# KTH-RPL/HiMo

Hardware: AMD Instinct MI355X
Metric: lidar_frames_per_sec_120k (higher is better)
Workload: dtype f16x2 (two-term split fp16, x = h + l with exact subnormals, on the matrix cores; float32 accumulate; ~22-bit products); 1 GPU; per-frame pipeline: pillarise 3 sweeps (512x512 grid) -> SeFlow++-style encoder/decoder + GRU head (random-init, self-specified: reference network source absent) -> per-point flow -> ego-motion removal + dt0 + flow2compDis -> comp_dis; points_per_frame=120000, sweeps_per_frame=3, parallelism=frames sharded x1, refined_output=False, batches_in_flight=3, matrix_arithmetic=f16x2, samples_per_backbone_launch=16, collectives=none (single process)

## Files before the change

### himo_amd/csrc/conv_common.h

```cpp
#pragma once
#include "himo_common.h"
#include "bf16x3.h"
#include <math.h>

namespace himo {

typedef float floatx16 __attribute__((ext_vector_type(16)));

enum Epilogue {
    kEpiBias = 0,
    kEpiBiasBnGelu = 1,
    kEpiBiasGelu = 2,
    kEpiGruZR = 3,
    kEpiGruQ = 4,
    kEpiBiasRelu = 5,
    kEpiReluMask = 6
};

struct ConvArgs {
    const float* x; int64_t x_batch_stride; int x_pitch;
    const float* w;
    const float* bias; const float* scale; const float* shift;
    float* y; int64_t y_batch_stride; int y_pitch;
    int N, H, W, Cin, Cout;
    int n_inner; int64_t x_outer_stride, y_outer_stride;
    int Ho, Wo;
    const float* aux_in; int aux_in_pitch;
    float* aux_out; int aux_out_pitch;
    int act_flags;
    unsigned* range_seen;
    const unsigned long long* mask;
    int64_t mask_batch_stride, mask_outer_stride;
};
enum ActFlags { kActSplitIn = 1, kActSplitOut = 2, kActVecStore = 4, kActAccumulate = 8, kActStuffedIn = 16, kActRowMask = 32 };

__device__ inline int64_t image_offset(int img, int n_inner, int64_t batch_stride, int64_t outer_stride) {
    return (int64_t)(img % n_inner) * batch_stride + (int64_t)(img / n_inner) * outer_stride;
}

__device__ inline int xcd_block_id(int bid, int n_blocks) {
    const int per = n_blocks >> 3, rem = n_blocks & 7;
    const int xcd = bid & 7, idx = bid >> 3;
    return xcd * per + (xcd < rem ? xcd : rem) + idx;
}

__device__ inline float gelu_exact(float v) {
    const float hv = 0.5f * v;
    const float t = __builtin_amdgcn_rcpf(fmaf(0.3275911f * 0.70710678118654752440f, fabsf(v), 1.0f));
    float p = fmaf(1.061405429f, t, -1.453152027f);
    p = fmaf(p, t, 1.421413741f);
    p = fmaf(p, t, -0.284496736f);
    p = fmaf(p, t, 0.254829592f);
    const float ex = __builtin_amdgcn_exp2f((v * v) * (-0.5f * 1.44269504088896340736f));
    const float e = fmaf(-(p * t), ex, 1.0f);
    return fmaf(fabsf(hv), e, hv);
// ... 55 lines not shown

__device__ inline unsigned split_word(float v, bool odd);
template <int EPI, bool PAIRED>
__device__ inline void split_store(const ConvArgs& a, float* __restrict__ yout, int64_t pix, int co, float v, float sc, float sh) {
    if (EPI == kEpiBiasBnGelu) v = gelu_exact(v * sc + sh);
    else if (EPI == kEpiBiasGelu) v = gelu_exact(v);
    else if (EPI == kEpiBiasRelu) v = fmaxf(v, 0.f);
    if (PAIRED) {
        const bool odd = co & 1;
        unsigned* rec = reinterpret_cast<unsigned*>(yout + pix * a.y_pitch + (co & ~15));
        rec[(odd ? 8 : 0) + ((co & 15) >> 1)] = split_word(v, odd);
        return;
    }
    unsigned h, l;
    split2_rounded(v, h, l);
    {
        unsigned short* rec = reinterpret_cast<unsigned short*>(yout + pix * a.y_pitch + (co & ~15));
        rec[co & 15] = (unsigned short)h;
        rec[16 + (co & 15)] = (unsigned short)l;
    }
}

constexpr float kSplitRangeGuard = 0.015625f;
__device__ inline void note_range(const ConvArgs& a, float v) {
    if (a.range_seen && __ballot(fabsf(v) >= kSplitRangeGuard) != 0ull && (threadIdx.x & 63) == 0 &&
        __hip_atomic_load(a.range_seen, __ATOMIC_RELAXED, __HIP_MEMORY_SCOPE_AGENT) == 0u)
        __hip_atomic_store(a.range_seen, 1u, __ATOMIC_RELAXED, __HIP_MEMORY_SCOPE_AGENT);
}

inline bool vec_store_ok(const ConvArgs& a) {
    return (reinterpret_cast<uintptr_t>(a.y) & 15u) == 0 && !(a.y_pitch & 3) && !(a.y_batch_stride & 3) && !(a.y_outer_stride & 3) && !(a.Cout & 3) &&
           (int64_t)a.Ho * a.Wo * a.y_pitch < ((int64_t)1 << 29);
}

template <bool OSPLIT, bool MASK = false, bool ACC = false>
__device__ inline void store_block_vec(const ConvArgs& a, float* __restrict__ yout, unsigned char* stg, const unsigned (&word)[16],
                                       int lane, int64_t pix0, int n_valid_px, int ch0) {
    const int li = lane & 31, lh = lane >> 5;
    const int widx = OSPLIT ? (li >> 4) * 16 + ((li & 1) ? 8 : 0) + ((li & 15) >> 1) : li;
#pragma unroll
    for (int r = 0; r < 16; ++r) {
        const int px = (r & 3) + 8 * (r >> 2) + 4 * lh;
        const int slot = px ^ ((px >> 2) & 1);
        *reinterpret_cast<unsigned*>(stg + slot * 128 + widx * 4) = word[r];
    }
    __builtin_amdgcn_wave_barrier();
#pragma unroll
    for (int t = 0; t < 4; ++t) {
        const int q = t * 64 + lane;
        const int slot = q >> 3, piece = q & 7;
        const int px = slot ^ ((slot >> 2) & 1);
// ... 34 lines not shown
```

### himo_amd/csrc/conv_plan.h

```cpp
#pragma once
#include "conv_common.h"

namespace himo {

enum ConvFamily {
    kConvF32,
    kConvStaged,
    kConvFromL2,
    kConvPresplit3,
    kConvPresplit1
};

struct ConvPlan {
    ConvFamily family;
    ConvArgs args;
    int ks, stride, epi, fmt;
    int bn, mi, ph, nt;
    const void* w_packed;
    dim3 grid;
    const char* prof_name;
};

void launch_conv_f32(const ConvPlan& p, hipStream_t s);
void launch_conv_staged(const ConvPlan& p, hipStream_t s);
void launch_conv_from_l2(const ConvPlan& p, hipStream_t s);
void launch_conv_presplit3(const ConvPlan& p, hipStream_t s);
void launch_conv_presplit1(const ConvPlan& p, hipStream_t s);

inline int64_t blocks_for(const ConvArgs& a, int th, int tw, int bn) {
    const int64_t tiles = th ? (int64_t)((a.Ho + th - 1) / th) * ((a.Wo + tw - 1) / tw) : ((int64_t)a.Ho * a.Wo + tw - 1) / tw;
    return (int64_t)a.N * tiles * ((a.Cout + bn - 1) / bn);
}

inline bool below_2gb(int64_t pixels, int pitch) { return pixels * pitch * 4 < ((int64_t)1 << 31); }

inline const char* conv_prof_name(int ks, int stride, int fmt) {
    static const char* const names[3][4] = {
        {"conv1x1_mfma_kernel", "conv1x1_bf16x3_kernel", "conv1x1_f16x2_kernel", "conv1x1_bf16x2_kernel"},
        {"conv3x3_mfma_kernel", "conv3x3_bf16x3_kernel", "conv3x3_f16x2_kernel", "conv3x3_bf16x2_kernel"},
        {"conv3x3s2_mfma_kernel", "conv3x3s2_bf16x3_kernel", "conv3x3s2_f16x2_kernel", "conv3x3s2_bf16x2_kernel"}};
    return names[ks == 1 ? 0 : stride == 2 ? 2 : 1][fmt < 0 ? 0 : fmt == 1 ? 2 : fmt == 2 ? 3 : 1];
}

// ... 38 lines not shown
    if (vec && (!(a.act_flags & kActSplitOut) || !(a.Cout & 15))) a.act_flags |= kActVecStore;
    return true;
}

inline int plan_presplit(ConvPlan& p, int rows_hint) {
    ConvArgs& a = p.args;
    if (!below_2gb((int64_t)a.H * a.W, a.x_pitch)) return HIMO_ERR_UNSUPPORTED;
    if (a.act_flags & kActRowMask) {
        p.family = kConvPresplit3;
        p.prof_name = "conv3x3_masked_f16x2_kernel";
        plan_rows_tile(p, 4, 2, 2);
        return HIMO_OK;
    }
    const bool wide = a.Cout > 64, vec = vec_store_ok(a), pinned = rows_hint == 4 || rows_hint == 2 || rows_hint == 1;
    const int ph = wide ? 1 : 2;
    p.family = p.ks == 1 ? kConvPresplit1 : kConvPresplit3;
    p.prof_name = conv_prof_name(p.ks, p.stride, 1);
    if (vec) a.act_flags |= kActVecStore;
    if (p.ks == 1) {
        int mi = wide ? 4 : 2;
        while (mi > 1 && blocks_for(a, 0, mi * ph * 32, (4 / ph) * 32) < 2048) mi >>= 1;
        if (pinned) mi = rows_hint;
        plan_rows_tile(p, ph, !wide && mi == 4 ? 2 : mi, 1);
    } else if (p.stride == 2) {
        plan_rows_tile(p, ph, wide ? 2 : 1, 1);
    } else if (!wide && rows_hint == 8 && vec) {
        plan_rows_tile(p, 4, 2, 2);
    } else if (wide && rows_hint == 12 && vec) {
        plan_rows_tile(p, a.Cout % 256 == 0 ? 1 : 2, 4, 2);
    } else {
        int mi = blocks_for(a, 4 * ph, 32, (4 / ph) * 32) >= 1024 ? 4 : 2;
        if (pinned) mi = rows_hint;
        plan_rows_tile(p, ph, !wide && mi == 4 ? 2 : mi, 1);
    }
    return HIMO_OK;
}

inline int plan_conv(const himo_conv_desc& d, ConvPlan& p) {
    if (!d.x || !d.w || !d.y) return HIMO_ERR_INVALID_ARGUMENT;
    if (d.n < 1 || d.h < 1 || d.w_in < 1 || d.cin < 1 || d.cout < 1) return HIMO_ERR_INVALID_ARGUMENT;
    if (!(d.ksize == 1 || d.ksize == 3) || !(d.stride == 1 || d.stride == 2)) return HIMO_ERR_UNSUPPORTED;
    if (d.ksize == 1 && d.stride != 1) return HIMO_ERR_UNSUPPORTED;
    if (d.epilogue < 0 || d.epilogue > kEpiReluMask) return HIMO_ERR_INVALID_ARGUMENT;
    if (d.epilogue == kEpiBiasBnGelu && (!d.scale || !d.shift)) return HIMO_ERR_INVALID_ARGUMENT;
    const bool gru = d.epilogue == kEpiGruZR || d.epilogue == kEpiGruQ;
    if (gru && (!d.aux_in || !d.aux_out)) return HIMO_ERR_INVALID_ARGUMENT;
// ... 22 lines not shown
            d.cout > 64 || (d.w_in & 31) || (d.epilogue != kEpiBias && d.epilogue != kEpiBiasBnGelu) || (d.cin & 15) || (d.x_pitch & 15))
            return HIMO_ERR_UNSUPPORTED;
        a.mask = reinterpret_cast<const unsigned long long*>(d.d_mask);
        a.mask_batch_stride = d.mask_batch_stride; a.mask_outer_stride = d.mask_outer_stride;
    }
    const bool gemm_acc = d.act_layout == kActAccumulate && d.w_packed && d.ksize == 1 && d.epilogue == kEpiBias && (d.packed_format == 0 || d.packed_format == 2);
    if (d.act_layout & (kActAccumulate | kActStuffedIn)) {
        if (!gemm_acc && ((d.act_layout & ~(kActAccumulate | kActStuffedIn)) || !d.w_packed || d.packed_format != 2 || d.ksize != 3 ||
                          d.stride != 1 || d.epilogue != kEpiBias))
            return HIMO_ERR_UNSUPPORTED;
        if ((d.act_layout & kActStuffedIn) && ((d.h & 1) || (d.w_in & 1) || !below_2gb((int64_t)(d.h / 2) * (d.w_in / 2), d.x_pitch)))
            return HIMO_ERR_UNSUPPORTED;
    } else if (d.act_layout && !(d.act_layout & kActRowMask)) {
        if ((d.act_layout & ~(kActSplitIn | kActSplitOut)) || !d.w_packed || d.packed_format != 1) return HIMO_ERR_UNSUPPORTED;
        if (d.ksize == 1 && !(d.act_layout & kActSplitIn)) return HIMO_ERR_UNSUPPORTED;
        if (d.epilogue != kEpiBias && d.epilogue != kEpiBiasBnGelu) return HIMO_ERR_UNSUPPORTED;
        if (((d.act_layout & kActSplitIn) && ((d.cin & 15) || (d.x_pitch & 15))) ||
            ((d.act_layout & kActSplitOut) && ((d.cout & 15) || (d.y_pitch & 15))))
            return HIMO_ERR_UNSUPPORTED;
    }

    const int hint = d.tile_hint, rows_hint = hint & 15;
    const bool l2_hint = hint == 0 || (hint & 0x1000);
    if (!d.w_packed || (d.stride == 2 && (gru || !l2_hint))) {
        p.family = kConvF32;
        plan_staged_tile(p, 4, 16, d.epilogue == kEpiGruZR, hint);
        p.prof_name = conv_prof_name(d.ksize, d.stride, -1);
        if (d.ksize == 1 && vec_store_ok(a) && !(a.Cout & 31) && (d.epilogue != kEpiReluMask || (aligned16(a.aux_in) && !(a.aux_in_pitch & 3))))
            a.act_flags |= kActVecStore;
        return HIMO_OK;
    }
    if (a.act_flags & kActSplitIn) return plan_presplit(p, rows_hint);
    const bool gemm_accumulate = gemm_acc && (int64_t)a.Ho * a.Wo * a.y_pitch < (1ll << 30);
    const bool from_l2 = d.ksize == 3 && l2_hint;
    if (a.act_flags && !gemm_accumulate && !from_l2) return HIMO_ERR_UNSUPPORTED;
    if (from_l2 && plan_from_l2(p, rows_hint)) return HIMO_OK;
    if (d.ksize == 3 && (hint & 0x1000) && rows_hint > 4) return HIMO_ERR_UNSUPPORTED;
    if (d.stride != 1) return HIMO_ERR_UNSUPPORTED;
    if (!below_2gb((int64_t)a.H * a.W, a.x_pitch)) return HIMO_ERR_UNSUPPORTED;
    if (d.packed_format == 2 && (d.ksize != 1 || (d.epilogue != kEpiBias && d.epilogue != kEpiReluMask) || (a.act_flags && !gemm_accumulate)))
        return HIMO_ERR_UNSUPPORTED;
    p.family = kConvStaged;
    plan_staged_tile(p, 2, 32, false, hint);
    p.prof_name = conv_prof_name(d.ksize, 1, d.packed_format);
    return HIMO_OK;
}
// ... 3 lines not shown
```

### himo_amd/csrc/convsg.hip

```cpp
#include "conv_plan.h"
#include "bf16x3.h"
#include <type_traits>

namespace himo {

__device__ __attribute__((aligned(64))) unsigned char g_zero_page[64];


__device__ inline void glds16(const void* gsrc, unsigned lds_dst) {
    unsigned keep;
    asm volatile("s_mov_b32 %0, m0\n\ts_mov_b32 m0, %2\n\ts_nop 0\n\tglobal_load_lds_dwordx4 %1, off\n\ts_mov_b32 m0, %0"
                 : "=&s"(keep) : "v"(gsrc), "s"(lds_dst) : "memory");
}

template <int EPI, int PH, int MI, bool OSPLIT, int S, int NT = 1>
__global__ __launch_bounds__(256, NT == 2 ? (MI == 2 ? 3 : 2) : (S == 2 || MI == 4) ? 3 : 4)
void conv3_presplit_kernel(ConvArgs a, const unsigned short* __restrict__ wpk) {
    constexpr int TW = 32, TH = MI * PH, PHt = S == 1 ? TH + 2 : 2 * TH + 1, PWP = S == 1 ? 40 : 80, UPR = PWP / 16;
    constexpr int kRow = PWP * 64, kBuf = (PHt * kRow + 1023) / 1024 * 1024;
    constexpr int kUnits = S == 1 ? (PHt * PWP + 15) / 16 : PHt * UPR, kUPW = (kUnits + 3) / 4;
    constexpr int BN = (4 / PH) * 32 * NT;
    __shared__ __attribute__((aligned(1024))) unsigned char patch[2 * kBuf];

    const int n_tiles_n = (a.Cout + BN - 1) / BN;
// ... 137 lines not shown
                for (int r = 0; r < 16; ++r) {
                    const float v = epi_activate<EPI>(acc[mi][nt][r], eA[nt], eB[nt]);
                    word[r] = OSPLIT ? split_word(v, li & 1) : __builtin_bit_cast(unsigned, v);
                    if (OSPLIT && mi == 0 && nt == 0 && r == 0)
                        note_range(a, (oy < a.Ho && 4 * lh < n_px && tn * BN + wc * NT * 32 + li < a.Cout) ? v : 0.f);
                }
                store_block_vec<OSPLIT>(a, yout, stg, word, lane, (int64_t)oy * a.Wo + ox0, oy < a.Ho ? n_px : 0, tn * BN + (wc * NT + nt) * 32);
            }
        }
        return;
    }
    if (!co_ok) return;
#pragma unroll
    for (int mi = 0; mi < MI; ++mi) {
        const int oy = oy0 + wp * MI + mi;
#pragma unroll
        for (int r = 0; r < 16; ++r) {
            const int ox = ox0 + (r & 3) + 8 * (r >> 2) + 4 * lh;
            if (oy < a.Ho && ox < a.Wo) {
                const float v = epi_activate<EPI>(acc[mi][0][r], eA[0], eB[0]);
                if (OSPLIT) split_store<kEpiBias, true>(a, yout, (int64_t)oy * a.Wo + ox, co, v, 1.f, 0.f);
                else yout[((int64_t)oy * a.Wo + ox) * a.y_pitch + co] = v;
            }
        }
    }
}

template <int EPI>
__global__ __launch_bounds__(256, 3)
void conv3_rowmask_kernel(ConvArgs a, const unsigned short* __restrict__ wpk) {
    constexpr int TW = 32, TH = 8, PHt = TH + 2, PWP = 40;
    constexpr int kRow = PWP * 64, kBuf = (PHt * kRow + 1023) / 1024 * 1024;
    static_assert(PHt * PWP == 25 * 16 && kBuf == 25 * 1024, "25 DMA units of 16 slots fill a patch buffer exactly");
    __shared__ __attribute__((aligned(1024))) unsigned char patch[2 * kBuf];
    __shared__ __attribute__((aligned(16))) unsigned char s_list[TH * TW];

    const int tile = xcd_block_id(blockIdx.x, gridDim.x);
    int bid = tile;
    const int tx = a.Wo / TW, ty = (a.Ho + TH - 1) / TH;
    const int ox0 = __builtin_amdgcn_readfirstlane((bid % tx) * TW); bid /= tx;
    const int oy0 = __builtin_amdgcn_readfirstlane((bid % ty) * TH);
    const int img = __builtin_amdgcn_readfirstlane(bid / ty);
    const int wave = __builtin_amdgcn_readfirstlane(threadIdx.x >> 6), lane = threadIdx.x & 63;
    const int li = lane & 31, lh = lane >> 5;

    const unsigned* __restrict__ mrow = reinterpret_cast<const unsigned*>(a.mask + image_offset(img, a.n_inner, a.mask_batch_stride, a.mask_outer_stride));
// ... 325 lines not shown

template <int PH, int MI, int S = 1, int NT = 1>
static void launch_sg(const ConvPlan& p, hipStream_t s) { HIMO_SG_EPI(conv3_presplit_kernel, S, NT); }
#undef HIMO_SG_EPI
#undef HIMO_SG

void launch_conv_presplit1(const ConvPlan& p, hipStream_t s) {
    if (p.ph == 1) {
        if (p.mi == 4) launch_sg1<1, 4>(p, s);
        else if (p.mi == 2) launch_sg1<1, 2>(p, s);
        else launch_sg1<1, 1>(p, s);
    } else {
        if (p.mi == 2) launch_sg1<2, 2>(p, s);
        else launch_sg1<2, 1>(p, s);
    }
}

void launch_conv_presplit3(const ConvPlan& p, hipStream_t s) {
    if (p.args.act_flags & kActRowMask) {
        if (p.epi == kEpiBias) hipLaunchKernelGGL((conv3_rowmask_kernel<kEpiBias>), p.grid, dim3(256), 0, s, p.args, (const unsigned short*)p.w_packed);
        else hipLaunchKernelGGL((conv3_rowmask_kernel<kEpiBiasBnGelu>), p.grid, dim3(256), 0, s, p.args, (const unsigned short*)p.w_packed);
        return;
    }
    if (p.stride == 2) { if (p.ph == 1) launch_sg<1, 2, 2>(p, s); else launch_sg<2, 1, 2>(p, s); }
    else if (p.nt == 2) {
        if (p.ph == 4) launch_sg<4, 2, 1, 2>(p, s);
        else if (p.ph == 1) launch_sg<1, 4, 1, 2>(p, s);
        else launch_sg<2, 4, 1, 2>(p, s);
    }
    else if (p.ph == 1) {
        if (p.mi == 4) launch_sg<1, 4>(p, s);
        else if (p.mi == 2) launch_sg<1, 2>(p, s);
        else launch_sg<1, 1>(p, s);
    } else {
        if (p.mi == 2) launch_sg<2, 2>(p, s);
        else launch_sg<2, 1>(p, s);
    }
}

}
```

### himo_amd/pipeline.py

```python
from __future__ import annotations

from dataclasses import dataclass

import numpy as np
import torch

from . import _lib
from .compdis import CompDisEngine, FrameBatch
from .seflow.model import SeFlowNet


@dataclass
class Sample:
    pch1: torch.Tensor
    pc0: torch.Tensor
    pc1: torch.Tensor
    pose_h1: np.ndarray
    pose0: np.ndarray
    pose1: np.ndarray
    lidar_dt: torch.Tensor
    scene_id: str = ""
    timestamp: int = 0

    @classmethod
# ... 58 lines not shown
        if F:
            torch.cat([s.pc0 for s in samples], dim=0, out=pc0)
            torch.cat([s.lidar_dt for s in samples], dim=0, out=dt)
        self._batch = FrameBatch(
            offsets_host=offsets, offsets=meta_dev[:o_end].view(torch.int64),
            pose0=meta_dev[o_end:o_end + p_len].view(torch.float64).view(F, 4, 4),
            pose1=meta_dev[o_end + p_len:o_end + 2 * p_len].view(torch.float64).view(F, 4, 4),
            pc0=pc0, lidar_dt=dt, flow=self._rows("flow", T, 3),
            meta=[(s.scene_id, s.timestamp) for s in samples])
        return self._batch

    def _forward(self, samples, outs) -> None:
        mb = self.net.max_batch
        for lo in range(0, len(samples), mb):
            grp = samples[lo:lo + mb]
            self.net.forward_batch([(s.pch1, s.pc0, s.pc1, s.pose_h1, s.pose0, s.pose1) for s in grp], outs[lo:lo + mb])

    def _set_sparse_dec4(self):
        net = self.net
        if hasattr(net, "sparse_dec4"):
            net.sparse_dec4 = bool(net.precision == "f16x2" and net.fused_head and net.split_acts)
            if hasattr(net, "head_offsets_only"):
                net.head_offsets_only = net.sparse_dec4

    def _fall_back(self):
        self.net = SeFlowNet(precision="bf16x3", **self._net_args)
        self._set_sparse_dec4()

    def _guard_begin(self):
        if self.net.precision == "f16x2":
            if not self.net.fused_head:
                raise RuntimeError("precision='f16x2' needs the fused head: its output stage carries the finite-flow guard")
            self.net.clear_nonfinite()

    def _guard_now(self) -> bool:
        if self.net.precision != "f16x2":
            return True
        self._guard_why = self.net.guard_verdict(self.net.guard.cpu().tolist())
        return self._guard_why is None

    def _guard_later(self):
        if self.net.precision != "f16x2":
            return
        if not hasattr(self, "_flag_ring"):
            self._flag_ring, self._flag_next = [torch.zeros(self.net.guard.numel(), dtype=torch.int32).pin_memory() for _ in range(2)], 0
        host = self._flag_ring[self._flag_next]
# ... 142 lines not shown
```

### himo_amd/seflow/model.py

```python
from __future__ import annotations

import ctypes

import numpy as np
import torch

from .. import _lib
from . import spec

EPI_BIAS, EPI_BIAS_BN_GELU, EPI_BIAS_GELU, EPI_GRU_ZR, EPI_GRU_Q = range(5)


class ConvDesc(ctypes.Structure):
    _fields_ = [("x", ctypes.c_void_p), ("x_batch_stride", ctypes.c_int64), ("x_pitch", ctypes.c_int),
                ("w", ctypes.c_void_p), ("bias", ctypes.c_void_p), ("scale", ctypes.c_void_p), ("shift", ctypes.c_void_p),
                ("y", ctypes.c_void_p), ("y_batch_stride", ctypes.c_int64), ("y_pitch", ctypes.c_int),
                ("n", ctypes.c_int), ("h", ctypes.c_int), ("w_in", ctypes.c_int), ("cin", ctypes.c_int),
                ("cout", ctypes.c_int), ("ksize", ctypes.c_int), ("stride", ctypes.c_int), ("epilogue", ctypes.c_int),
                ("aux_in", ctypes.c_void_p), ("aux_in_pitch", ctypes.c_int),
                ("aux_out", ctypes.c_void_p), ("aux_out_pitch", ctypes.c_int), ("w_packed", ctypes.c_void_p),
                ("tile_hint", ctypes.c_int), ("packed_format", ctypes.c_int),
                ("n_outer", ctypes.c_int), ("x_outer_stride", ctypes.c_int64), ("y_outer_stride", ctypes.c_int64),
                ("act_layout", ctypes.c_int), ("range_seen", ctypes.c_void_p),
                ("mask", ctypes.c_void_p), ("mask_batch_stride", ctypes.c_int64), ("mask_outer_stride", ctypes.c_int64)]


ACT_SPLIT_IN, ACT_SPLIT_OUT = 1, 2
ACT_ROW_MASK = 32
ACT_ACCUMULATE = 8
ACT_STUFFED_2X = 16
PILLAR_NO_LISTS, PILLAR_HALFWAVE_ONLY = 4, 8


_lib.register({
    "himo_pillar_workspace_bytes": (ctypes.c_size_t, [ctypes.c_int64, ctypes.c_int, ctypes.c_int]),
    "himo_pillar_occupancy_reset": (ctypes.c_int, [ctypes.c_void_p, ctypes.c_size_t, ctypes.c_int, ctypes.c_int, ctypes.c_void_p]),
    "himo_pillarize": (ctypes.c_int, [ctypes.c_int64, ctypes.c_void_p, ctypes.c_int, ctypes.POINTER(ctypes.c_float),
                                      ctypes.POINTER(ctypes.c_float), ctypes.POINTER(ctypes.c_float),
                                      ctypes.POINTER(ctypes.c_float), ctypes.c_int, ctypes.c_int,
                                      ctypes.c_void_p, ctypes.c_void_p, ctypes.c_void_p,
                                      ctypes.c_void_p, ctypes.c_void_p, ctypes.c_void_p, ctypes.c_void_p,
                                      ctypes.c_int, ctypes.c_void_p, ctypes.c_size_t, ctypes.c_void_p]),
    "himo_conv2d": (ctypes.c_int, [ctypes.POINTER(ConvDesc), ctypes.c_void_p]),
    "himo_conv_packed_weight_bytes": (ctypes.c_size_t, [ctypes.c_int, ctypes.c_int, ctypes.c_int]),
    "himo_conv_pack_weights": (ctypes.c_int, [ctypes.c_void_p, ctypes.c_int, ctypes.c_int, ctypes.c_int, ctypes.c_void_p,
                                              ctypes.c_void_p]),
    "himo_upsample2x": (ctypes.c_int, [ctypes.c_void_p, ctypes.c_int, ctypes.c_int, ctypes.c_int, ctypes.c_int,
# ... 80 lines not shown

class SeFlowNet:

    def __init__(self, params: dict | None = None, device=None, max_points: int = 140_000, seed: int = 0,
                 precision: str = "bf16x3", autotune: bool = True, max_batch: int = 1):
        if precision not in ("bf16x3", "f16x2", "f32"):
            raise ValueError(precision)
        if max_batch < 1:
            raise ValueError("max_batch")
        self.max_batch = max_batch
        self.precision = precision
        self.autotune = autotune
        self.keep_cell_lists = False
        self.fused_head = precision != "f32"
        self._incremental_images = True
        self.use_plan = True
        self.use_graph = True
        self._plans = {}
        self._recording = None
        self._nb = 1
        self.packed_format = 1 if precision == "f16x2" else 0
        self._split_acts = precision == "f16x2"
        self._sparse_dec4 = False
        self.head_offsets_only = False
        self.tiles = {}
        self.lib = _lib.load()
        self.device = device if device is not None else _lib.require_gpu()
        params = spec.init_params(seed) if params is None else params
        shapes = spec.param_shapes()
        for k, shp in shapes.items():
            if k not in params or tuple(params[k].shape) != tuple(shp):
                raise KeyError(f"parameter {k} missing or of wrong shape (want {shp})")
        cpu = {k: torch.from_numpy(np.ascontiguousarray(params[k], dtype=np.float32)) for k in shapes}
        def fold(prefix, eps):
            scale = cpu[f"{prefix}.gamma"] / torch.sqrt(cpu[f"{prefix}.var"] + eps)
            return scale, cpu[f"{prefix}.beta"] - cpu[f"{prefix}.mean"] * scale
        derived = {}
        derived["pfn.scale"], derived["pfn.shift"] = fold("pfn.bn", spec.BN_EPS_PFN)
        for name, *_ in spec.ENCODER:
            derived[f"{name}.scale"], derived[f"{name}.shift"] = fold(f"{name}.bn", spec.BN_EPS)
        self.fold_decoder = True
        for a, b in (("dec1", "dec2"), ("dec2", "dec3")):
            w5, b5 = cpu[f"{a}.u5.weight"].double().numpy(), cpu[f"{a}.u5.bias"].double().numpy()
            w1, b1 = cpu[f"{b}.u1.weight"].double().numpy()[0, 0], cpu[f"{b}.u1.bias"].double().numpy()
            derived[f"{a}.u5>{b}.u1.weight"] = torch.from_numpy(np.ascontiguousarray(w5 @ w1, dtype=np.float32))
            derived[f"{a}.u5>{b}.u1.bias"] = torch.from_numpy(np.ascontiguousarray(b5 @ w1 + b1, dtype=np.float32))
# ... 83 lines not shown

    @property
    def incremental_images(self) -> bool:
        return self._incremental_images

    @incremental_images.setter
    def incremental_images(self, on: bool):
        on = bool(on)
        if on != self._incremental_images:
            self._incremental_images = on
            self.reset_images()

    @property
    def split_acts(self) -> bool:
        return self._split_acts

    @split_acts.setter
    def split_acts(self, on: bool):
        on = bool(on)
        if on != self._split_acts:
            self._split_acts = on
            if not on:
                self._sparse_dec4 = False
            self.drop_plan()
            self.reset_images()

    HEAD_SLOT = 1

    @property
    def sparse_dec4(self) -> bool:
        return self._sparse_dec4

    @sparse_dec4.setter
    def sparse_dec4(self, on: bool):
        on = bool(on)
        if on and not (self.packed_format == 1 and self._split_acts and self.fused_head):
            raise ValueError("sparse_dec4 needs precision='f16x2' with split activations and the fused head")
        if on != self._sparse_dec4:
            self._sparse_dec4 = on
            self.drop_plan()

    @property
    def B0(self):
        return self._B0

    @B0.setter
    def B0(self, buf):
        self._B0 = buf
        self.drop_plan()
        self.reset_images()

    MAX_RANGE_SLOTS = 63

    def clear_nonfinite(self):
        _lib.check(self.lib.himo_clear_u32(self.guard.data_ptr(), self.guard.numel(), _lib.stream_handle()), "himo_clear_u32")

    def _range_word(self, wname: str) -> int:
        k = self._range_slots.setdefault(wname, len(self._range_slots))
        if k >= self.MAX_RANGE_SLOTS:
            raise RuntimeError("more split-output layers than guard words")
        return self.guard.data_ptr() + 4 * (1 + k)

    def guard_verdict(self, words) -> str | None:
        w = [int(v) for v in words]
        if w[0] != 0:
            return "overflow"
        if w[-1] != 0 and any(w[1 + k] == 0 for k in self._range_slots.values()):
            return "underflow"
        return None

    def reset_images(self):
        for st in getattr(self, "_pt", ()):
            for ws in st["ws_slots"]:
                _lib.check(self.lib.himo_pillar_occupancy_reset(ws.data_ptr(), ws.numel(), self.W, self.H, _lib.stream_handle()),
                           "himo_pillar_occupancy_reset")

    def _use_sample(self, i: int):
        st = self._pt[i]
        self._sample = i
        self.ws_slots, self.xyz_t, self.pid, self.offsets = st["ws_slots"], st["xyz_t"], st["pid"], st["offsets"]

    def _conv(self, x, x_bs, x_pitch, wname, y, y_bs, y_pitch, n, h, w, cin, cout, ks, stride, epi, x_off=0, y_off=0,
              scale=None, shift=None, aux_in=None, aux_in_pitch=0, aux_out=None, aux_out_pitch=0, bias=None, batched=True,
              act=0, mask=None):
        d = ConvDesc()
        d.x = x.data_ptr() + 4 * x_off; d.x_batch_stride = x_bs; d.x_pitch = x_pitch
        if batched and self._nb > 1:
            d.n_outer, d.x_outer_stride, d.y_outer_stride = self._nb, x.stride(0), y.stride(0)
        d.w = self.p[f"{wname}.weight"].data_ptr()
        d.bias = (self.p[f"{wname}.bias"] if bias is None else bias).data_ptr()
        d.scale = None if scale is None else scale.data_ptr()
        d.shift = None if shift is None else shift.data_ptr()
        d.y = y.data_ptr() + 4 * y_off; d.y_batch_stride = y_bs; d.y_pitch = y_pitch
        d.n, d.h, d.w_in, d.cin, d.cout, d.ksize, d.stride, d.epilogue = n, h, w, cin, cout, ks, stride, epi
        d.aux_in = None if aux_in is None else aux_in.data_ptr(); d.aux_in_pitch = aux_in_pitch
        d.aux_out = None if aux_out is None else aux_out.data_ptr(); d.aux_out_pitch = aux_out_pitch
        pk = self.packed.get(f"{wname}.weight")
        d.w_packed = None if pk is None else pk.data_ptr()
        d.packed_format = self.packed_format
        d.act_layout = act if self.split_acts else 0
        if mask is not None:
            d.act_layout |= ACT_ROW_MASK
            d.mask, d.mask_batch_stride, d.mask_outer_stride = mask.data_ptr(), 0, mask.stride(0)
        if (d.act_layout & ACT_SPLIT_OUT) and self.packed_format == 1 and epi in (EPI_BIAS, EPI_BIAS_BN_GELU):
            d.range_seen = self._range_word(wname)
        key = (n * max(d.n_outer, 1), h, w, cin, cout, ks, stride, epi, pk is not None, d.act_layout)
        if self.autotune and key not in self.tiles:
            self.tiles[key] = self._tune(d)
        d.tile_hint = self.tiles.get(key, 0)
        if self._recording is not None and epi not in (EPI_GRU_ZR, EPI_GRU_Q):
            op = HimoOp(); op.kind = 0; op.conv = d
            self._recording.append(op)
        _lib.check(self.lib.himo_conv2d(ctypes.byref(d), _lib.stream_handle()), f"himo_conv2d({wname})")

    def _tune(self, d: "ConvDesc") -> int:
        if d.epilogue in (EPI_GRU_ZR, EPI_GRU_Q) or (d.act_layout & ACT_ROW_MASK):
            return 0
        cands = [(bn << 4) | mi for bn in (128, 64) if not (bn == 128 and d.cout % 128) for mi in (2, 1)]
        if d.act_layout:
            if d.stride == 2 and (d.act_layout & ACT_SPLIT_IN):
                return 0
            cands = [0x1000 | 4, 0x1000 | 2, 0x1000 | 1] if d.ksize == 1 else []
        if d.w_packed and d.ksize == 3:
            cands += [0x1000 | 4, 0x1000 | 2, 0x1000 | 1] if d.stride == 1 else [0x1000 | 2, 0x1000 | 1]
            if d.stride == 1 and (d.act_layout & ACT_SPLIT_IN) and self.packed_format == 1:
                cands.append(0x1000 | (8 if d.cout <= 64 else 12))
        if len(cands) < 2:
            return cands[0] if cands else 0
        return fastest_tile_hint(self.lib, d, cands, warmup=2)
# ... 25 lines not shown
        self.encoder()
        self.decoder()
        if self._recording is not None:
            rec, self._recording = self._recording, None
            self._plans[n_samples] = ((HimoOp * len(rec))(*rec), len(rec))
        return self.DEC

    def __del__(self):
        try:
            self.drop_plan()
        except Exception:
            pass

    def drop_plan(self):
        for plan in self._plans.values():
            self.lib.himo_ops_release(ctypes.addressof(plan[0]))
        self._plans = {}

    def encoder(self):
        H, W, F = self.H, self.W, self.F
        p = self.p
        stages = [("enc1", 4, 32, 64, H, W, self.E1, self.F1), ("enc2", 6, 64, 128, H // 2, W // 2, self.E2, self.F2),
                  ("enc3", 6, 128, 256, H // 4, W // 4, self.E3, self.F3)]
        src, src_bs, src_pitch = self.B0, 32, 32 * F
        for stage, n_conv, cin, cout, h, w, pingpong, catbuf in stages:
            ho, wo = h // 2, w // 2
            for i in range(n_conv):
                name = f"{stage}.{i}"
                last = i == n_conv - 1
                dst = catbuf if last else pingpong[i % 2]
                dst_bs, dst_pitch = (cout, cout * F) if last else (ho * wo * cout, cout)
                act = ACT_SPLIT_IN | ACT_SPLIT_OUT
                if i == 0:
                    self._conv(src, src_bs, src_pitch, name, dst, dst_bs, dst_pitch, F, h, w, cin, cout, 3, 2,
                               EPI_BIAS_BN_GELU, scale=p[f"{name}.scale"], shift=p[f"{name}.shift"], act=act)
                else:
                    self._conv(src, src_bs, src_pitch, name, dst, dst_bs, dst_pitch, F, ho, wo, cout, cout, 3, 1,
                               EPI_BIAS_BN_GELU, scale=p[f"{name}.scale"], shift=p[f"{name}.shift"], act=act)
                src, src_bs, src_pitch = dst, dst_bs, dst_pitch

    def decoder(self):
        H, W, F = self.H, self.W, self.F
        IN, IO = ACT_SPLIT_IN, ACT_SPLIT_IN | ACT_SPLIT_OUT
        fold = self.fold_decoder
        def block(name, coarse, c_in, ch, cw, tmp, cat, skip, skip_c, lat, out, work, nxt=None):
            if coarse is not None:
                self._conv(coarse, 0, c_in, f"{name}.u1", tmp, 0, lat, 1, 1, ch * cw, c_in, lat, 1, 1, EPI_BIAS, act=IN)
            self._up(tmp, lat, ch, cw, lat, cat, 2 * lat, out_split=True)
            self._conv(skip, 0, skip_c, f"{name}.u3", cat, 0, 2 * lat, 1, 1, 4 * ch * cw, skip_c, lat, 1, 1, EPI_BIAS, y_off=lat, act=IO)
            self._conv(cat, 0, 2 * lat, f"{name}.u4", work[0], 0, out, 1, 2 * ch, 2 * cw, 2 * lat, out, 3, 1, EPI_BIAS, act=IO)
            if fold and nxt is not None:
                nname, ntmp, nlat = nxt
                self._conv(work[0], 0, out, f"{name}.u5>{nname}.u1", ntmp, 0, nlat, 1, 2 * ch, 2 * cw, out, nlat, 3, 1, EPI_BIAS, act=IN)
                return None
            self._conv(work[0], 0, out, f"{name}.u5", work[1], 0, out, 1, 2 * ch, 2 * cw, out, out, 3, 1, EPI_BIAS, act=IO)
            return work[1]
        s = block("dec1", self.F3, 256 * F, H // 8, W // 8, self.T1, self.CAT1, self.F2, 128 * F, 256, 256, self.S, ("dec2", self.T2, 128))
        t = block("dec2", s, 256, H // 4, W // 4, self.T2, self.CAT2, self.F1, 64 * F, 128, 128, self.T, ("dec3", self.T3, 64))
        u = block("dec3", t, 128, H // 2, W // 2, self.T3, self.CAT3, self.B0, 32 * F, 64, 64, self.U)
        self._conv(u, 0, 64, "dec4", self.DEC, 0, 64, 1, H, W, 64, 64, 3, 1, EPI_BIAS, act=IN,
                   mask=self.occ0 if self._sparse_dec4 else None)
        return self.DEC

    def head(self, pc0: torch.Tensor, slot0: int = 1, slot1: int = 2, out: torch.Tensor | None = None) -> torch.Tensor:
        n = pc0.shape[0]
        p = self.p
        F = self.F
        B0, DEC = self.B0[self._sample], self.DEC[self._sample]
        if self.fused_head:
            flow = out if out is not None else torch.empty((n, 3), dtype=torch.float32, device=self.device)
            if flow.shape != (n, 3) or flow.dtype != torch.float32 or not flow.is_contiguous():
                raise ValueError("out must be a contiguous (N0,3) float32 tensor")
# ... 201 lines not shown
```

### include/himo_amd.h

```cpp
#ifndef HIMO_AMD_H
#define HIMO_AMD_H

#include <stddef.h>
#include <stdint.h>

#ifdef __cplusplus
extern "C" {
#endif

#define HIMO_ABI_VERSION 1

typedef enum himo_status {
    HIMO_OK = 0,
    HIMO_ERR_INVALID_ARGUMENT = 1,
    HIMO_ERR_EMPTY_FRAME = 2,
    HIMO_ERR_WORKSPACE = 3,
    HIMO_ERR_SINGULAR_POSE = 4,
    HIMO_ERR_HIP = 5,
    HIMO_ERR_UNSUPPORTED = 6
} himo_status;

#define HIMO_FLAG_F32_CHAIN 0x1u
#define HIMO_FLAG_RAW 0x2u
#define HIMO_FLAG_SCANIA 0x4u
// ... 307 lines not shown
#define HIMO_EPI_BIAS_BN_GELU 1
#define HIMO_EPI_BIAS_GELU 2
#define HIMO_EPI_GRU_ZR 3
#define HIMO_EPI_GRU_Q 4
#define HIMO_EPI_BIAS_RELU 5
#define HIMO_EPI_RELU_MASK 6
typedef struct himo_conv_desc {
    const float* x; int64_t x_batch_stride; int x_pitch;
    const float* w;
    const float* bias; const float* scale; const float* shift;
    float* y; int64_t y_batch_stride; int y_pitch;
    int n, h, w_in, cin, cout, ksize, stride, epilogue;
    const float* aux_in; int aux_in_pitch;
    float* aux_out; int aux_out_pitch;
    const void* w_packed;
    int tile_hint;
    int packed_format;
    int n_outer;
    int64_t x_outer_stride, y_outer_stride;
    int act_layout;
    uint32_t* d_range_seen;
    const uint64_t* d_mask;
    int64_t mask_batch_stride, mask_outer_stride;
} himo_conv_desc;
#define HIMO_ACT_SPLIT_IN 1
#define HIMO_ACT_SPLIT_OUT 2
#define HIMO_ACT_ROW_MASK 32
#define HIMO_ACT_ACCUMULATE 8
#define HIMO_ACT_STUFFED_2X 16
int himo_conv2d(const himo_conv_desc* h_desc, void* stream);
size_t himo_conv_packed_weight_bytes(int ksize, int cin, int cout);
int himo_conv_pack_weights(const float* d_w, int ksize, int cin, int cout, void* d_packed, void* stream);
#define HIMO_PACK_BF16X3 0
#define HIMO_PACK_F16X2 1
#define HIMO_PACK_BF16X2 2
int himo_conv_pack_weights_ex(const float* d_w, int ksize, int cin, int cout, int format, void* d_packed, void* stream);

int himo_upsample2x(const float* d_x, int x_pitch, int h, int w, int c, float* d_y, int y_pitch, void* stream);
int himo_upsample2x_batch(int n, const float* d_x, int64_t x_batch_stride, int x_pitch, int h, int w, int c, float* d_y,
                          int64_t y_batch_stride, int y_pitch, void* stream);
int himo_upsample2x_batch_ex(int n, const float* d_x, int64_t x_batch_stride, int x_pitch, int h, int w, int c, float* d_y,
                             int64_t y_batch_stride, int y_pitch, int out_split, void* stream);

#define HIMO_OP_CONV 0
#define HIMO_OP_UPSAMPLE2X 1
#define HIMO_OPS_GRAPH 0x1u
// ... 275 lines not shown
```

Baseline: 772.2 frames/s.

## Fuse decoder skip 1x1 conv into enc1 stride-2 conv kernel

Adds a fused stride-2 3x3 conv kernel that also computes the dec3 skip 1x1 projection (u3) from the same staged input patch, producing the full-resolution skip output while the encoder conv runs. The separate u3 launch for dec3 is removed when fused_skips is enabled, which is turned on by default for f16x2 with split activations. This saves a kernel launch and a second full read of the input, at the cost of extra MFMA work, extra accumulator registers, and scattered 4-byte stores in the fused kernel. The grid is divided by 3 because each block loops over all three sweep frames.

```diff
diff --git a/himo_amd/csrc/conv_common.h b/himo_amd/csrc/conv_common.h
--- a/himo_amd/csrc/conv_common.h
+++ b/himo_amd/csrc/conv_common.h
@@ -31,6 +31,13 @@
     unsigned* range_seen;
     const unsigned long long* mask;
     int64_t mask_batch_stride, mask_outer_stride;
+};
+struct SkipArgs {
+    const unsigned short* w;
+    const float* bias;
+    float* y; int y_pitch; int64_t y_outer_stride;
+    int cout;
+    unsigned* range_seen;
 };
 enum ActFlags { kActSplitIn = 1, kActSplitOut = 2, kActVecStore = 4, kActAccumulate = 8, kActStuffedIn = 16, kActRowMask = 32 };
 
@@ -132,11 +139,12 @@
 }
 
 constexpr float kSplitRangeGuard = 0.015625f;
-__device__ inline void note_range(const ConvArgs& a, float v) {
-    if (a.range_seen && __ballot(fabsf(v) >= kSplitRangeGuard) != 0ull && (threadIdx.x & 63) == 0 &&
-        __hip_atomic_load(a.range_seen, __ATOMIC_RELAXED, __HIP_MEMORY_SCOPE_AGENT) == 0u)
-        __hip_atomic_store(a.range_seen, 1u, __ATOMIC_RELAXED, __HIP_MEMORY_SCOPE_AGENT);
-}
+__device__ inline void note_range(unsigned* range_seen, float v) {
+    if (range_seen && __ballot(fabsf(v) >= kSplitRangeGuard) != 0ull && (threadIdx.x & 63) == 0 &&
+        __hip_atomic_load(range_seen, __ATOMIC_RELAXED, __HIP_MEMORY_SCOPE_AGENT) == 0u)
+        __hip_atomic_store(range_seen, 1u, __ATOMIC_RELAXED, __HIP_MEMORY_SCOPE_AGENT);
+}
+__device__ inline void note_range(const ConvArgs& a, float v) { note_range(a.range_seen, v); }
 
 inline bool vec_store_ok(const ConvArgs& a) {
     return (reinterpret_cast<uintptr_t>(a.y) & 15u) == 0 && !(a.y_pitch & 3) && !(a.y_batch_stride & 3) && !(a.y_outer_stride & 3) && !(a.Cout & 3) &&
diff --git a/himo_amd/csrc/conv_plan.h b/himo_amd/csrc/conv_plan.h
--- a/himo_amd/csrc/conv_plan.h
+++ b/himo_amd/csrc/conv_plan.h
@@ -19,6 +19,8 @@
     const void* w_packed;
     dim3 grid;
     const char* prof_name;
+    bool fused;
+    SkipArgs skip;
 };
 
 void launch_conv_f32(const ConvPlan& p, hipStream_t s);
@@ -103,6 +105,11 @@
         while (mi > 1 && blocks_for(a, 0, mi * ph * 32, (4 / ph) * 32) < 2048) mi >>= 1;
         if (pinned) mi = rows_hint;
         plan_rows_tile(p, ph, !wide && mi == 4 ? 2 : mi, 1);
+    } else if (p.stride == 2 && p.fused) {
+        if (!vec) return HIMO_ERR_UNSUPPORTED;
+        plan_rows_tile(p, 2, 1, 1);
+        p.grid.x /= 3;
+        p.prof_name = "conv3x3s2_skip_f16x2_kernel";
     } else if (p.stride == 2) {
         plan_rows_tile(p, ph, wide ? 2 : 1, 1);
     } else if (!wide && rows_hint == 8 && vec) {
@@ -171,6 +178,20 @@
 
     const int hint = d.tile_hint, rows_hint = hint & 15;
     const bool l2_hint = hint == 0 || (hint & 0x1000);
+    if (d.skip_w_packed || d.skip_bias || d.skip_y || d.skip_y_pitch || d.skip_y_outer_stride || d.skip_cout || d.skip_d_range_seen) {
+        if (!d.skip_w_packed || !d.skip_y) return HIMO_ERR_INVALID_ARGUMENT;
+        if (d.ksize != 3 || d.stride != 2 || d.act_layout != (kActSplitIn | kActSplitOut) || !l2_hint || (d.h & 1) || (d.w_in & 1) ||
+            d.n != 3 || d.x_batch_stride != d.cin || d.x_pitch < 3 * d.cin ||
+            d.skip_cout < 16 || (d.skip_cout & 15) || d.skip_cout > (d.cout + 63) / 64 * 64 ||
+            d.skip_y_pitch < d.skip_cout || (d.skip_y_pitch & 15) || (d.skip_y_outer_stride & 15) ||
+            (reinterpret_cast<uintptr_t>(d.skip_y) & 63u) || (int64_t)d.h * d.w_in * d.skip_y_pitch >= ((int64_t)1 << 29))
+            return HIMO_ERR_UNSUPPORTED;
+        p.fused = true;
+        p.skip.w = static_cast<const unsigned short*>(d.skip_w_packed); p.skip.bias = d.skip_bias;
+        p.skip.y = d.skip_y; p.skip.y_pitch = d.skip_y_pitch; p.skip.y_outer_stride = d.skip_y_outer_stride;
+        p.skip.cout = d.skip_cout; p.skip.range_seen = d.skip_d_range_seen;
+    }
+
     if (!d.w_packed || (d.stride == 2 && (gru || !l2_hint))) {
         p.family = kConvF32;
         plan_staged_tile(p, 4, 16, d.epilogue == kEpiGruZR, hint);
diff --git a/himo_amd/csrc/convsg.hip b/himo_amd/csrc/convsg.hip
--- a/himo_amd/csrc/convsg.hip
+++ b/himo_amd/csrc/convsg.hip
@@ -183,6 +183,184 @@
                 if (OSPLIT) split_store<kEpiBias, true>(a, yout, (int64_t)oy * a.Wo + ox, co, v, 1.f, 0.f);
                 else yout[((int64_t)oy * a.Wo + ox) * a.y_pitch + co] = v;
             }
+        }
+    }
+}
+
+template <int EPI>
+__global__ __launch_bounds__(256, 3)
+void conv3s2_skip_kernel(ConvArgs a, const unsigned short* __restrict__ wpk, SkipArgs k) {
+    constexpr int TW = 32, TH = 2, PHt = 2 * TH + 1, PWP = 80, UPR = PWP / 16;
+    constexpr int kRow = PWP * 64, kBuf = (PHt * kRow + 1023) / 1024 * 1024;
+    constexpr int BN = 64;
+    static_assert(UPR == 5 && PHt == 5 && kBuf >= 4 * 4096, "the epilogue's four wave-private 4 KB corners fit one patch buffer");
+    __shared__ __attribute__((aligned(1024))) unsigned char patch[2 * kBuf];
+
+    const int n_tiles_n = (a.Cout + BN - 1) / BN;
+    int bid = xcd_block_id(blockIdx.x, gridDim.x);
+    const int tn = bid % n_tiles_n; bid /= n_tiles_n;
+    const int tx = (a.Wo + TW - 1) / TW, ty = (a.Ho + TH - 1) / TH;
+    const int ox0 = (bid % tx) * TW; bid /= tx;
+    const int oy0 = (bid % ty) * TH;
+    const int smp = bid / ty;
+    const unsigned char* __restrict__ xin = reinterpret_cast<const unsigned char*>(a.x + (int64_t)smp * a.x_outer_stride);
+    const int slabs = a.Cin >> 4, steps = 3 * slabs;
+
+    const int wave = __builtin_amdgcn_readfirstlane(threadIdx.x >> 6), lane = threadIdx.x & 63;
+    const int wp = wave & 1, wc = wave >> 1;
+    const int li = lane & 31, lh = lane >> 5;
+    const int ct = tn * BN + wc * 32;
+    const int iy0 = oy0 * 2 - 1, ix0 = ox0 * 2 - 1;
+    const unsigned lds_base = (unsigned)(uintptr_t)(__attribute__((address_space(3))) unsigned char*)(&patch[0]);
+
+    unsigned offA, offB, vm = 0u;
+    const unsigned rs = (unsigned)a.W * (unsigned)a.x_pitch * 4u;
+    {
+        const int px = wave * 16 + (lane >> 2), col = px < 48 ? 2 * px : 2 * (px - 48) + 1, ix = ix0 + col;
+        const bool col_ok = (px <= 32 || px >= 48) && ix >= 0 && ix < a.W;
+        offA = (((unsigned)(iy0 * a.W + ix) * (unsigned)a.x_pitch) << 2) | (unsigned)(((lane & 3) ^ ((px >> 2) & 3)) << 4);
+#pragma unroll
+        for (int r = 0; r < PHt; ++r) vm |= (col_ok && iy0 + r >= 0 && iy0 + r < a.H) ? 1u << r : 0u;
+    }
+    {
+        const int px = 64 + (lane >> 2), ix = ix0 + 2 * (px - 48) + 1, row = wave;
+        const bool col_ok = ix >= 0 && ix < a.W;
+        offB = (((unsigned)((iy0 + row) * a.W + ix) * (unsigned)a.x_pitch) << 2) | (unsigned)(((lane & 3) ^ ((px >> 2) & 3)) << 4);
+        vm |= (col_ok && iy0 + row >= 0 && iy0 + row < a.H) ? 1u << 5 : 0u;
+        vm |= (wave == 0 && col_ok && iy0 + 4 >= 0 && iy0 + 4 < a.H) ? 1u << 6 : 0u;
+    }
+    auto stage = [&](int step, int buf) {
+        int ln = threadIdx.x;
+        unsigned oa = offA, ob = offB, m = vm;
+        asm volatile("" : "+v"(ln), "+v"(oa), "+v"(ob), "+v"(m));
+        const unsigned char* zero = g_zero_page + (ln & 3) * 16;
+        const unsigned dst = lds_base + buf * kBuf;
+#pragma unroll
+        for (int r = 0; r < PHt; ++r)
+            glds16((m >> r) & 1u ? xin + (oa + r * rs + (unsigned)step * 64u) : zero, dst + r * kRow + wave * 1024);
+        glds16((m >> 5) & 1u ? xin + (ob + (unsigned)step * 64u) : zero, dst + wave * kRow + 4 * 1024);
+        if (wave == 0) glds16((m >> 6) & 1u ? xin + (ob + 4 * rs + (unsigned)step * 64u) : zero, dst + 4 * kRow + 4 * 1024);
+    };
+
+    floatx16 acc, acc1[4];
+#pragma unroll
+    for (int r = 0; r < 16; ++r) { acc[r] = 0.f; acc1[0][r] = 0.f; acc1[1][r] = 0.f; acc1[2][r] = 0.f; acc1[3][r] = 0.f; }
+
+    const unsigned char* __restrict__ wb = reinterpret_cast<const unsigned char*>(wpk);
+    const unsigned b_lane = (unsigned)(ct + li < a.Cout ? ct + li : a.Cout - 1) * 32u + (unsigned)lh * 16u;
+    const unsigned b_plane = (unsigned)a.Cout * 32u, b_block = 2u * b_plane;
+    auto load_b = [&](int tap, int slab, uint4 (&b)[2]) {
+        const unsigned off = (unsigned)(tap * slabs + slab) * b_block + b_lane;
+        b[0] = *reinterpret_cast<const uint4*>(wb + off);
+        b[1] = *reinterpret_cast<const uint4*>(wb + (off + b_plane));
+    };
+    const unsigned char* __restrict__ wb1 = reinterpret_cast<const unsigned char*>(k.w);
+    const unsigned b1_lane = (unsigned)(ct + li < k.cout ? ct + li : k.cout - 1) * 32u + (unsigned)lh * 16u;
+    const unsigned b1_plane = (unsigned)k.cout * 32u;
+    auto load_b1 = [&](int step, uint4 (&b)[2]) {
+        const unsigned off = (unsigned)step * (2u * b1_plane) + b1_lane;
+        b[0] = *reinterpret_cast<const uint4*>(wb1 + off);
+        b[1] = *reinterpret_cast<const uint4*>(wb1 + (off + b1_plane));
+    };
+
+    int rd[3][2];
+#pragma unroll
+    for (int kx = 0; kx < 3; ++kx) {
+        const int p = (kx & 1) * 48 + li + (kx >> 1), f = (p >> 2) & 3;
+#pragma unroll
+        for (int s = 0; s < 2; ++s) rd[kx][s] = wp * 2 * kRow + p * 64 + (((2 * s + lh) ^ f) << 4);
+    }
+
+    uint4 bq[3][2], b1[2];
+    stage(0, 0);
+    load_b(0, 0, bq[0]);
+    load_b(1, 0, bq[1]);
+    load_b1(0, b1);
+    asm volatile("s_waitcnt vmcnt(0)" ::: "memory");
+    __syncthreads();
+
+    int slab = 0, frame = 0;
+#pragma unroll 1
+    for (int step = 0; step < steps; ++step) {
+        const int buf = step & 1;
+        const bool more = step + 1 < steps;
+        const bool last_of_frame = slab + 1 == slabs;
+        const int nslab = last_of_frame ? 0 : slab + 1;
+        if (more) stage(step + 1, buf ^ 1);
+#pragma unroll
+        for (int ky = 0; ky < 3; ++ky) {
+            const int rowoff = buf * kBuf + ky * kRow;
+#pragma unroll
+            for (int kx = 0; kx < 3; ++kx) {
+                const int tap = ky * 3 + kx;
+                const int t2 = tap + 2;
+                constexpr int kNone = -1;
+                const int j1 = (ky >= 1 && kx >= 1) ? 2 * (ky - 1) + (kx - 1) : kNone;
+                load_b(t2 < 9 ? t2 : t2 - 9, t2 < 9 ? slab : nslab, bq[(tap + 2) % 3]);
+                f16x8 af[2];
+#pragma unroll
+                for (int s = 0; s < 2; ++s) af[s] = *reinterpret_cast<const f16x8*>(&patch[rd[kx][s] + rowoff]);
+                const uint4 (&bcur)[2] = bq[tap % 3];
+#define HIMO_TERM16(SA, SB)                                                                                                  \
+    acc = __builtin_amdgcn_mfma_f32_32x32x16_f16(af[SA], __builtin_bit_cast(f16x8, bcur[SB]), acc, 0, 0, 0);                   \
+    if (j1 != kNone) acc1[j1 < 0 ? 0 : j1] = __builtin_amdgcn_mfma_f32_32x32x16_f16(af[SA], __builtin_bit_cast(f16x8, b1[SB]), acc1[j1 < 0 ? 0 : j1], 0, 0, 0);
+                { HIMO_TERM16(1, 0) HIMO_TERM16(0, 1) HIMO_TERM16(0, 0) }
+#undef HIMO_TERM16
+                __builtin_amdgcn_sched_group_barrier(0x020, 2, 0);
+                __builtin_amdgcn_sched_group_barrier(0x100, 2, 0);
+                if (j1 != kNone) __builtin_amdgcn_sched_group_barrier(0x008, 6, 0);
+                else __builtin_amdgcn_sched_group_barrier(0x008, 3, 0);
+            }
+        }
+        if (more) {
+            load_b1(step + 1, b1);
+            asm volatile("s_waitcnt vmcnt(6)" ::: "memory");
+            __syncthreads();
+        }
+        if (!last_of_frame) { ++slab; continue; }
+
+        if (!more) __syncthreads();
+        {
+            int ln = threadIdx.x;
+            asm volatile("" : "+v"(ln));
+            const int lane = ln & 63, li = ln & 31, lh = (ln >> 5) & 1;
+            float* __restrict__ yout = a.y + (int64_t)frame * a.y_batch_stride + (int64_t)smp * a.y_outer_stride;
+            const int c = ct + li < a.Cout ? ct + li : a.Cout - 1;
+            float eA, eB;
+            epi_affine<EPI>(kF16AccScale, a.bias ? a.bias[c] : 0.f, EPI == kEpiBiasBnGelu ? a.scale[c] : 1.f, EPI == kEpiBiasBnGelu ? a.shift[c] : 0.f, eA, eB);
+            unsigned char* stg = patch + buf * kBuf + wave * 4096;
+            const int n_px = a.Wo - ox0 < 32 ? a.Wo - ox0 : 32;
+            const int oy = oy0 + wp;
+            unsigned word[16];
+#pragma unroll
+            for (int r = 0; r < 16; ++r) {
+                const float v = epi_activate<EPI>(acc[r], eA, eB);
+                word[r] = split_word(v, li & 1);
+                if (r == 0) note_range(a, (oy < a.Ho && 4 * lh < n_px && ct + li < a.Cout) ? v : 0.f);
+                acc[r] = 0.f;
+            }
+            store_block_vec<true>(a, yout, stg, word, lane, (int64_t)oy * a.Wo + ox0, oy < a.Ho ? n_px : 0, ct);
+        }
+        if (more) __syncthreads();
+        slab = 0; ++frame;
+    }
+
+    const int c1 = ct + li;
+    float eA, eB;
+    epi_affine<kEpiBias>(kF16AccScale, k.bias ? k.bias[c1 < k.cout ? c1 : k.cout - 1] : 0.f, 1.f, 0.f, eA, eB);
+    unsigned* __restrict__ y1 = reinterpret_cast<unsigned*>(k.y + (int64_t)smp * k.y_outer_stride);
+    const unsigned word_at = (unsigned)((c1 & ~15) + ((c1 & 1) ? 8 : 0) + ((c1 & 15) >> 1));
+#pragma unroll
+    for (int j = 0; j < 4; ++j) {
+        const int hy = 2 * (oy0 + wp) + (j >> 1);
+#pragma unroll
+        for (int r = 0; r < 16; ++r) {
+            const int hx = 2 * (ox0 + (r & 3) + 8 * (r >> 2) + 4 * lh) + (j & 1);
+            const bool ok = hy < a.H && hx < a.W && c1 < k.cout;
+            const float v = epi_activate<kEpiBias>(acc1[j][r], eA, eB);
+            const unsigned w = split_word(v, li & 1);
+            if (j == 0 && r == 0) note_range(k.range_seen, ok ? v : 0.f);
+            if (ok) y1[((unsigned)hy * (unsigned)a.W + (unsigned)hx) * (unsigned)k.y_pitch + word_at] = w;
         }
     }
 }
@@ -554,6 +732,11 @@
         else hipLaunchKernelGGL((conv3_rowmask_kernel<kEpiBiasBnGelu>), p.grid, dim3(256), 0, s, p.args, (const unsigned short*)p.w_packed);
         return;
     }
+    if (p.fused) {
+        if (p.epi == kEpiBias) hipLaunchKernelGGL((conv3s2_skip_kernel<kEpiBias>), p.grid, dim3(256), 0, s, p.args, (const unsigned short*)p.w_packed, p.skip);
+        else hipLaunchKernelGGL((conv3s2_skip_kernel<kEpiBiasBnGelu>), p.grid, dim3(256), 0, s, p.args, (const unsigned short*)p.w_packed, p.skip);
+        return;
+    }
     if (p.stride == 2) { if (p.ph == 1) launch_sg<1, 2, 2>(p, s); else launch_sg<2, 1, 2>(p, s); }
     else if (p.nt == 2) {
         if (p.ph == 4) launch_sg<4, 2, 1, 2>(p, s);
diff --git a/himo_amd/pipeline.py b/himo_amd/pipeline.py
--- a/himo_amd/pipeline.py
+++ b/himo_amd/pipeline.py
@@ -104,6 +104,8 @@
             net.sparse_dec4 = bool(net.precision == "f16x2" and net.fused_head and net.split_acts)
             if hasattr(net, "head_offsets_only"):
                 net.head_offsets_only = net.sparse_dec4
+        if hasattr(net, "fused_skips"):
+            net.fused_skips = bool(net.precision == "f16x2" and net.split_acts)
 
     def _fall_back(self):
         self.net = SeFlowNet(precision="bf16x3", **self._net_args)
diff --git a/himo_amd/seflow/model.py b/himo_amd/seflow/model.py
--- a/himo_amd/seflow/model.py
+++ b/himo_amd/seflow/model.py
@@ -22,7 +22,10 @@
                 ("tile_hint", ctypes.c_int), ("packed_format", ctypes.c_int),
                 ("n_outer", ctypes.c_int), ("x_outer_stride", ctypes.c_int64), ("y_outer_stride", ctypes.c_int64),
                 ("act_layout", ctypes.c_int), ("range_seen", ctypes.c_void_p),
-                ("mask", ctypes.c_void_p), ("mask_batch_stride", ctypes.c_int64), ("mask_outer_stride", ctypes.c_int64)]
+                ("mask", ctypes.c_void_p), ("mask_batch_stride", ctypes.c_int64), ("mask_outer_stride", ctypes.c_int64),
+                ("skip_w_packed", ctypes.c_void_p), ("skip_bias", ctypes.c_void_p), ("skip_y", ctypes.c_void_p),
+                ("skip_y_pitch", ctypes.c_int), ("skip_y_outer_stride", ctypes.c_int64), ("skip_cout", ctypes.c_int),
+                ("skip_range_seen", ctypes.c_void_p)]
 
 
 ACT_SPLIT_IN, ACT_SPLIT_OUT = 1, 2
@@ -149,6 +152,7 @@
         self.packed_format = 1 if precision == "f16x2" else 0
         self._split_acts = precision == "f16x2"
         self._sparse_dec4 = False
+        self._fused_skips = False
         self.head_offsets_only = False
         self.tiles = {}
         self.lib = _lib.load()
@@ -278,6 +282,7 @@
             self._split_acts = on
             if not on:
                 self._sparse_dec4 = False
+                self._fused_skips = False
             self.drop_plan()
             self.reset_images()
 
@@ -296,6 +301,21 @@
             self._sparse_dec4 = on
             self.drop_plan()
 
+    FUSED_SKIP_STAGES = {"enc1": "dec3"}
+
+    @property
+    def fused_skips(self) -> bool:
+        return self._fused_skips
+
+    @fused_skips.setter
+    def fused_skips(self, on: bool):
+        on = bool(on)
+        if on and not (self.packed_format == 1 and self._split_acts):
+            raise ValueError("fused_skips needs precision='f16x2' with split activations")
+        if on != self._fused_skips:
+            self._fused_skips = on
+            self.drop_plan()
+
     @property
     def B0(self):
         return self._B0
@@ -338,7 +358,7 @@
 
     def _conv(self, x, x_bs, x_pitch, wname, y, y_bs, y_pitch, n, h, w, cin, cout, ks, stride, epi, x_off=0, y_off=0,
               scale=None, shift=None, aux_in=None, aux_in_pitch=0, aux_out=None, aux_out_pitch=0, bias=None, batched=True,
-              act=0, mask=None):
+              act=0, mask=None, skip=None):
         d = ConvDesc()
         d.x = x.data_ptr() + 4 * x_off; d.x_batch_stride = x_bs; d.x_pitch = x_pitch
         if batched and self._nb > 1:
@@ -360,7 +380,12 @@
             d.mask, d.mask_batch_stride, d.mask_outer_stride = mask.data_ptr(), 0, mask.stride(0)
         if (d.act_layout & ACT_SPLIT_OUT) and self.packed_format == 1 and epi in (EPI_BIAS, EPI_BIAS_BN_GELU):
             d.range_seen = self._range_word(wname)
-        key = (n * max(d.n_outer, 1), h, w, cin, cout, ks, stride, epi, pk is not None, d.act_layout)
+        if skip is not None:
+            sname, sy, d.skip_y_pitch, s_off, d.skip_cout = skip
+            d.skip_w_packed, d.skip_bias = self.packed[f"{sname}.weight"].data_ptr(), self.p[f"{sname}.bias"].data_ptr()
+            d.skip_y, d.skip_y_outer_stride = sy.data_ptr() + 4 * s_off, sy.stride(0)
+            d.skip_range_seen = self._range_word(sname)
+        key = (n * max(d.n_outer, 1), h, w, cin, cout, ks, stride, epi, pk is not None, d.act_layout, skip is not None)
         if self.autotune and key not in self.tiles:
             self.tiles[key] = self._tune(d)
         d.tile_hint = self.tiles.get(key, 0)
@@ -432,6 +457,7 @@
         p = self.p
         stages = [("enc1", 4, 32, 64, H, W, self.E1, self.F1), ("enc2", 6, 64, 128, H // 2, W // 2, self.E2, self.F2),
                   ("enc3", 6, 128, 256, H // 4, W // 4, self.E3, self.F3)]
+        skips = {"enc1": (self.CAT3, 64), "enc2": (self.CAT2, 128), "enc3": (self.CAT1, 256)} if self._fused_skips else {}
         src, src_bs, src_pitch = self.B0, 32, 32 * F
         for stage, n_conv, cin, cout, h, w, pingpong, catbuf in stages:
             ho, wo = h // 2, w // 2
@@ -442,8 +468,12 @@
                 dst_bs, dst_pitch = (cout, cout * F) if last else (ho * wo * cout, cout)
                 act = ACT_SPLIT_IN | ACT_SPLIT_OUT
                 if i == 0:
+                    skip = None
+                    if stage in skips and stage in self.FUSED_SKIP_STAGES:
+                        cat, lat = skips[stage]
+                        skip = (f"{self.FUSED_SKIP_STAGES[stage]}.u3", cat, 2 * lat, lat, lat)
                     self._conv(src, src_bs, src_pitch, name, dst, dst_bs, dst_pitch, F, h, w, cin, cout, 3, 2,
-                               EPI_BIAS_BN_GELU, scale=p[f"{name}.scale"], shift=p[f"{name}.shift"], act=act)
+                               EPI_BIAS_BN_GELU, scale=p[f"{name}.scale"], shift=p[f"{name}.shift"], act=act, skip=skip)
                 else:
                     self._conv(src, src_bs, src_pitch, name, dst, dst_bs, dst_pitch, F, ho, wo, cout, cout, 3, 1,
                                EPI_BIAS_BN_GELU, scale=p[f"{name}.scale"], shift=p[f"{name}.shift"], act=act)
@@ -457,7 +487,8 @@
             if coarse is not None:
                 self._conv(coarse, 0, c_in, f"{name}.u1", tmp, 0, lat, 1, 1, ch * cw, c_in, lat, 1, 1, EPI_BIAS, act=IN)
             self._up(tmp, lat, ch, cw, lat, cat, 2 * lat, out_split=True)
-            self._conv(skip, 0, skip_c, f"{name}.u3", cat, 0, 2 * lat, 1, 1, 4 * ch * cw, skip_c, lat, 1, 1, EPI_BIAS, y_off=lat, act=IO)
+            if not (self._fused_skips and name in self.FUSED_SKIP_STAGES.values()):
+                self._conv(skip, 0, skip_c, f"{name}.u3", cat, 0, 2 * lat, 1, 1, 4 * ch * cw, skip_c, lat, 1, 1, EPI_BIAS, y_off=lat, act=IO)
             self._conv(cat, 0, 2 * lat, f"{name}.u4", work[0], 0, out, 1, 2 * ch, 2 * cw, 2 * lat, out, 3, 1, EPI_BIAS, act=IO)
             if fold and nxt is not None:
                 nname, ntmp, nlat = nxt
diff --git a/include/himo_amd.h b/include/himo_amd.h
--- a/include/himo_amd.h
+++ b/include/himo_amd.h
@@ -353,6 +353,10 @@
     uint32_t* d_range_seen;
     const uint64_t* d_mask;
     int64_t mask_batch_stride, mask_outer_stride;
+    const void* skip_w_packed; const float* skip_bias;
+    float* skip_y; int skip_y_pitch; int64_t skip_y_outer_stride;
+    int skip_cout;
+    uint32_t* skip_d_range_seen;
 } himo_conv_desc;
 #define HIMO_ACT_SPLIT_IN 1
 #define HIMO_ACT_SPLIT_OUT 2
```

Result: no change. 770.7 frames/s (-0.2%).
